# yahoo/bftkv

Measured on AMD Instinct MI355X. Metric: pgp_rsa2048_signature_verifies_per_sec, higher is better.
Workload: dtype u32; 1 GPU; 64-replica quorum, 10000 RSA-2048 signed writes per GPU (cfg2 of BASELINE.json), 534164 signature packets per GPU, 1.0% corrupt / 0.5% unknown issuer / 0.5% duplicate / 1.0% one-short; parallelism=shard-by-write x1, RCCL all-gather of verdict bitmaps on the verifier's stream, replicas=64, writes_per_gpu=10000, sigs_per_gpu=534164, batches_in_flight=3

## Files before the change

### bftkv_amd/csrc/kernels.hip

```cpp
#include <hip/hip_runtime.h>
#include <stdint.h>

#include "device_types.h"
#include "mont28.h"
#include "u256.h"
#include "hashes.h"

namespace bftkv {

struct ParsedPacket {
  uint64_t next;
  bool event;
  SigRec rec;
};

__host__ __device__ __forceinline__ bool known_tag(uint32_t tag) {
  return tag < 32 && ((0x00066BFEu >> tag) & 1u);
}

struct SubpacketState {
  bool have_ctime = false, have_issuer = false, have_embedded = false;
  bool too_deep = false;
  uint64_t issuer = 0;
};
// ... 829 lines not shown
    if (which == 0) sha224_init(s); else if (which == 1) sha1_init(s); else if (which == 4) md5_init(s); else ripemd160_init(s);
    for (uint64_t blk = 0; blk < (len >> 6); ++blk) {
      uint32_t w[16];
      if (which >= 4) { load_block_le(p + blk * 64, w); if (which == 4) md5_compress(s, w); else ripemd160_compress(s, w); }
      else { load_block_be(p + blk * 64, w); if (which == 0) sha256_compress(s, w); else sha1_compress(s, w); }
    }
    const uint32_t slot32 = which < 2 ? which + 1 : which - 1;
    uint32_t* o = mid32 + ((uint64_t)slot32 * n_items + item) * 8;
#pragma unroll
    for (int i = 0; i < 8; ++i) o[i] = s[i];
  } else {
    uint64_t s[8];
    if (which == 2) sha512_init(s); else sha384_init(s);
    for (uint64_t blk = 0; blk < (len >> 7); ++blk) {
      uint32_t lo[16], hi[16];
      load_block_be(p + blk * 128, lo);
      load_block_be(p + blk * 128 + 64, hi);
      uint64_t w[16];
#pragma unroll
      for (int i = 0; i < 8; ++i) { w[i] = ((uint64_t)lo[2 * i] << 32) | lo[2 * i + 1]; w[8 + i] = ((uint64_t)hi[2 * i] << 32) | hi[2 * i + 1]; }
      sha512_compress(s, w);
    }
    uint64_t* o = mid64 + ((uint64_t)(which - 2) * n_items + item) * 8;
#pragma unroll
    for (int i = 0; i < 8; ++i) o[i] = s[i];
  }
}

__global__ void __launch_bounds__(64) k_hash_mid_text(const uint8_t* __restrict__ tbs_blob, const uint64_t* __restrict__ tbs_off,
                                                      uint32_t n_items, const uint32_t* __restrict__ item_hash_mask, TextDev txt) {
  const uint32_t item = blockIdx.x * blockDim.x + threadIdx.x;
  const uint32_t which = blockIdx.y;
  if (item >= n_items) return;
  if (!((item_hash_mask[item] >> (ITEM_TEXT_SHIFT + which)) & 1u)) return;
  const uint8_t* p = tbs_blob + tbs_off[item];
  const uint64_t len = tbs_off[item + 1] - tbs_off[item];
  const bool wide = which == 3 || which == 4;
  const uint32_t B = wide ? 128u : 64u;
  uint32_t s32[8];
  uint64_t s64[8];
  if (which == 0) sha256_init(s32); else if (which == 1) sha224_init(s32); else if (which == 2) sha1_init(s32);
  else if (which == 3) sha512_init(s64); else if (which == 4) sha384_init(s64); else if (which == 5) md5_init(s32); else ripemd160_init(s32);
  uint8_t buf[128];
  uint32_t fill = 0;
  uint64_t total = 0;
  auto put = [&](uint8_t c) {
    buf[fill++] = c;
    ++total;
    if (fill == B) {
      if (which >= 5) {
        uint32_t w[16];
#pragma unroll
        for (int i = 0; i < 16; ++i) w[i] = (uint32_t)buf[4 * i] | ((uint32_t)buf[4 * i + 1] << 8) | ((uint32_t)buf[4 * i + 2] << 16) | ((uint32_t)buf[4 * i + 3] << 24);
        if (which == 5) md5_compress(s32, w); else ripemd160_compress(s32, w);
      } else if (!wide) {
        uint32_t w[16];
#pragma unroll
        for (int i = 0; i < 16; ++i) w[i] = ((uint32_t)buf[4 * i] << 24) | ((uint32_t)buf[4 * i + 1] << 16) | ((uint32_t)buf[4 * i + 2] << 8) | buf[4 * i + 3];
        if (which == 2) sha1_compress(s32, w); else sha256_compress(s32, w);
      } else {
        uint64_t w[16];
#pragma unroll
        for (int i = 0; i < 16; ++i) {
          uint64_t v = 0;
#pragma unroll
          for (int t = 0; t < 8; ++t) v = (v << 8) | buf[8 * i + t];
          w[i] = v;
        }
        sha512_compress(s64, w);
      }
      fill = 0;
    }
  };
  int st = 0;
  for (uint64_t i = 0; i < len; ++i) {
    const uint8_t c = p[i];
    if (st == 0) {
      if (c == 0x0D) { st = 1; put(c); }
      else if (c == 0x0A) { put(0x0D); put(0x0A); }
      else put(c);
    } else { st = 0; put(c); }
  }
  const uint64_t slot = (uint64_t)which * n_items + item;
  if (!wide) {
    const uint32_t slot32 = which < 3 ? which : which - 2;
    for (int i = 0; i < 8; ++i) txt.mid32[((uint64_t)slot32 * n_items + item) * 8 + i] = s32[i];
  } else { for (int i = 0; i < 8; ++i) txt.mid64[((uint64_t)(which - 3) * n_items + item) * 8 + i] = s64[i]; }
  for (uint32_t i = 0; i < fill; ++i) txt.tail[slot * 128 + i] = buf[i];
  txt.len[slot] = total;
}

struct TailSrc {
  const uint8_t* tail; uint32_t tail_len;
  const uint8_t* body; uint32_t pre_len;
  uint32_t tr_len;
  uint32_t rep;
};
__device__ __forceinline__ uint32_t tail_byte(const TailSrc& t, uint32_t j) {
  if (j < t.tail_len) return t.tail[j];
  j -= t.tail_len;
  const uint32_t unit = t.pre_len + t.tr_len;
  if (j >= unit * t.rep) return (j == unit * t.rep) ? 0x80 : 0;
  if (t.rep > 1) j %= unit;
  if (j < t.pre_len) return t.body[j];
  j -= t.pre_len;
  if (j == 0) return 0x04;
  if (j == 1) return 0xFF;
  return (t.pre_len >> (8 * (5 - j))) & 0xFF;
}

template <typename F>
__device__ __forceinline__ uint32_t limb28(F byte_from_lsb, int j) {
  uint32_t bit = 28u * (uint32_t)j;
  uint32_t b0 = bit >> 3, sh = bit & 7;
  uint64_t v = 0;
#pragma unroll
  for (int t = 0; t < 5; ++t) v |= (uint64_t)byte_from_lsb(b0 + t) << (8 * t);
  return (uint32_t)(v >> sh) & MONT_MASK;
}

template <bool OTHERS>
__device__ __forceinline__ void digest_body(const uint8_t* __restrict__ tbs_blob, const uint64_t* __restrict__ tbs_off,
                                            const uint8_t* __restrict__ sig_blob, const uint32_t* __restrict__ mid32,
                                            const uint64_t* __restrict__ mid64, uint32_t n_items,
                                            SigRec* __restrict__ recs, uint32_t n_recs, uint32_t* __restrict__ digests ,
                                            uint32_t ri_in, const uint64_t* __restrict__ tbs_prefix = nullptr, uint32_t rep = 1,
                                            uint32_t* __restrict__ tag_only = nullptr, TextDev txt = TextDev{nullptr, nullptr, nullptr, nullptr}) {
  const uint32_t ri = ri_in;
  if (ri >= n_recs) return;
  const SigRec rec = recs[ri];
  if (!tag_only && rec.status != ST_PENDING_HASH) return;
  const bool text = OTHERS && (rec.flags & SIGF_TEXT) != 0;
  if (!tag_only && ((rec.hash_id != HASH_SHA256) || (rec.flags & SIGF_TEXT) != 0) != OTHERS) return;
  if (OTHERS && text && !txt.len) return;
  const HashInfo hi = OTHERS ? hash_info(rec.hash_id) : HashInfo{32, 0, 32, 19};
  const uint64_t seg = tbs_off[rec.item + 1] - tbs_off[rec.item];
  const uint32_t bmask = (OTHERS && hi.family == 64) ? 127u : 63u;
  const uint64_t tslot = (uint64_t)hi.idx * n_items + rec.item;
  const uint64_t tlen = text ? txt.len[tslot] : (tbs_prefix ? tbs_prefix[rec.item] + seg : seg);
  TailSrc ts;
  ts.tail_len = text ? (uint32_t)(tlen & bmask) : (tbs_prefix ? (uint32_t)seg : (uint32_t)(tlen & bmask));
  ts.tail = text ? txt.tail + tslot * 128 : tbs_blob + tbs_off[rec.item] + (seg - ts.tail_len);
  const bool v3 = (rec.flags & SIGF_V3) != 0;
  ts.body = sig_blob + rec.body_off + (v3 ? 2 : 0);
  ts.pre_len = v3 ? 5u : 6u + rec.hashed_len;
  ts.tr_len = v3 ? 0u : 6u;
  ts.rep = rep;
  const uint32_t rem = ts.tail_len + (ts.pre_len + ts.tr_len) * rep;
  const uint64_t bits = (tlen + (uint64_t)(ts.pre_len + ts.tr_len) * rep) * 8;
  uint32_t dg_dummy[16];
  uint32_t* dg = tag_only ? dg_dummy : digests + (uint64_t)ri * 16;
  uint32_t tag_hi;
  if (!OTHERS || hi.family == 32) {
    const uint32_t nblk = (rem + 9 + 63) >> 6;
    uint32_t s[8];
    const uint32_t* m = (text ? txt.mid32 : mid32) + ((uint64_t)hi.slot * n_items + rec.item) * 8;
#pragma unroll
    for (int i = 0; i < 8; ++i) s[i] = m[i];
    const bool le = OTHERS && hi.le;
    for (uint32_t blk = 0; blk < nblk; ++blk) {
      uint32_t w[16];
#pragma unroll
      for (int i = 0; i < 16; ++i) {
        uint32_t j = blk * 64 + i * 4;
        const uint32_t be = (tail_byte(ts, j) << 24) | (tail_byte(ts, j + 1) << 16) | (tail_byte(ts, j + 2) << 8) | tail_byte(ts, j + 3);
        w[i] = le ? __builtin_bswap32(be) : be;
      }
      if (blk == nblk - 1) { w[14] = le ? (uint32_t)bits : (uint32_t)(bits >> 32); w[15] = le ? (uint32_t)(bits >> 32) : (uint32_t)bits; }
      if (OTHERS && hi.slot == 2) sha1_compress(s, w);
      else if (OTHERS && hi.slot == 3) md5_compress(s, w);
      else if (OTHERS && hi.slot == 4) ripemd160_compress(s, w);
      else sha256_compress(s, w);
    }
#pragma unroll
    for (int i = 0; i < 8; ++i) dg[i] = le ? s[i] : __builtin_bswap32(s[i]);
    tag_hi = le ? __builtin_bswap32(s[0]) : s[0];
  } else if (OTHERS) {
    const uint32_t nblk = (rem + 17 + 127) >> 7;
    uint64_t s[8];
    const uint64_t* m = (text ? txt.mid64 : mid64) + ((uint64_t)hi.slot * n_items + rec.item) * 8;
#pragma unroll
    for (int i = 0; i < 8; ++i) s[i] = m[i];
    for (uint32_t blk = 0; blk < nblk; ++blk) {
      uint64_t w[16];
#pragma unroll
      for (int i = 0; i < 16; ++i) {
        uint32_t j = blk * 128 + i * 8;
        uint64_t v = 0;
#pragma unroll
        for (int t = 0; t < 8; ++t) v = (v << 8) | tail_byte(ts, j + t);
        w[i] = v;
      }
      if (blk == nblk - 1) { w[14] = 0; w[15] = bits; }
      sha512_compress(s, w);
    }
#pragma unroll
    for (int i = 0; i < 8; ++i) { dg[2 * i] = __builtin_bswap32((uint32_t)(s[i] >> 32)); dg[2 * i + 1] = __builtin_bswap32((uint32_t)s[i]); }
    tag_hi = (uint32_t)(s[0] >> 32);
  } else {
    tag_hi = 0;
  }
  if (tag_only) { *tag_only = tag_hi >> 16; return; }
  uint8_t st;
  if ((uint8_t)(tag_hi >> 24) != rec.hash_tag[0] || (uint8_t)(tag_hi >> 16) != rec.hash_tag[1]) st = ST_HASH_TAG;
  else st = (rec.after_tag == AFTER_TAG_PUBKEY) ? (uint8_t)ST_PENDING_RSA : rec.after_tag;
  recs[ri].status = st;
}

__global__ void __launch_bounds__(256) k_digest_sha256(const uint8_t* __restrict__ tbs_blob, const uint64_t* __restrict__ tbs_off,
                                                       const uint8_t* __restrict__ sig_blob, const uint32_t* __restrict__ mid32,
                                                       const uint64_t* __restrict__ mid64, uint32_t n_items, SigRec* __restrict__ recs,
                                                       uint32_t n_recs, uint32_t* __restrict__ digests,
                                                       const uint64_t* __restrict__ tbs_prefix, const uint32_t* __restrict__ n_recs_dev) {
  digest_body<false>(tbs_blob, tbs_off, sig_blob, mid32, mid64, n_items, recs, n_recs_dev ? *n_recs_dev : n_recs, digests,
                     blockIdx.x * blockDim.x + threadIdx.x, tbs_prefix);
}
__global__ void __launch_bounds__(256) k_digest_other(const uint8_t* __restrict__ tbs_blob, const uint64_t* __restrict__ tbs_off,
                                                         const uint8_t* __restrict__ sig_blob, const uint32_t* __restrict__ mid32,
                                                         const uint64_t* __restrict__ mid64, uint32_t n_items, SigRec* __restrict__ recs,
                                                         uint32_t n_recs, uint32_t* __restrict__ digests,
                                                         const uint32_t* __restrict__ any_other , TextDev txt,
                                                         const uint32_t* __restrict__ n_recs_dev ) {
  if (*any_other == 0) return;
  if (n_recs_dev) n_recs = *n_recs_dev;
  for (uint64_t ri = (uint64_t)blockIdx.x * blockDim.x + threadIdx.x; ri < n_recs; ri += (uint64_t)gridDim.x * blockDim.x)
    digest_body<true>(tbs_blob, tbs_off, sig_blob, mid32, mid64, n_items, recs, n_recs, digests, (uint32_t)ri, nullptr, 1, nullptr, txt);
}

__global__ void __launch_bounds__(64) k_candidates(const uint8_t* __restrict__ tbs_blob, const uint64_t* __restrict__ tbs_off,
                                                   const uint8_t* __restrict__ sig_blob, const uint32_t* __restrict__ mid32,
                                                   const uint64_t* __restrict__ mid64, uint32_t n_items, SigRec* __restrict__ recs,
                                                   uint32_t n_recs, const uint32_t* __restrict__ n_recs_dev, const uint64_t* __restrict__ tbs_prefix,
                                                   KeyTableDev kt, const uint32_t* __restrict__ cert_ent, const uint8_t* __restrict__ sig_class,
                                                   TextDev txt, uint32_t* __restrict__ item_hash_mask) {
  const uint32_t ri = blockIdx.x * blockDim.x + threadIdx.x;
  const uint32_t nr = n_recs_dev ? *n_recs_dev : n_recs;
  if (ri >= nr) return;
  const SigRec rec = recs[ri];
  if (!(rec.flags & SIGF_MORE_CANDIDATES)) return;
  uint8_t st = rec.status;
  if (!(st == ST_KEY_CANNOT_SIGN || st == ST_HASH_TAG || st == ST_ALGO_MISMATCH || st == ST_BAD_SIG)) return;
  if (tbs_prefix && (rec.hash_id != HASH_SHA256 || (rec.flags & SIGF_TEXT))) return;
  const uint32_t slot = (uint32_t)rec.key_slot;
  const uint64_t issuer = kt.key_id[slot];
  const uint32_t only_ent = cert_ent ? cert_ent[rec.item] : 0xFFFFFFFFu;
  const uint32_t cls = sig_class ? sig_class[rec.item] : 0;
  uint32_t lo_i = 0, hi_i = kt.n_keys;
  while (lo_i < hi_i) {
    const uint32_t mid = (lo_i + hi_i) >> 1;
    if (kt.sorted_id[mid] < issuer) lo_i = mid + 1; else hi_i = mid;
  }
  bool behind = false;
  uint32_t writes = (kt.flags[slot] & KEYF_CAN_SIGN) ? 1u : 0u;
  for (uint32_t i = lo_i; i < kt.n_keys && kt.sorted_id[i] == issuer; ++i) {
    const uint32_t k = kt.sorted_slot[i];
    if (!key_is_candidate(kt, k, only_ent, cls)) continue;
    if (k == slot) { behind = true; continue; }
    if (!behind) continue;
    if (!(kt.flags[k] & KEYF_CAN_SIGN)) { st = ST_KEY_CANNOT_SIGN; continue; }
    ++writes;
    uint32_t tag = 0;
    if (rec.hash_id == HASH_SHA256 && !(rec.flags & SIGF_TEXT))
      digest_body<false>(tbs_blob, tbs_off, sig_blob, mid32, mid64, n_items, recs, nr, nullptr, ri, tbs_prefix, writes, &tag);
    else digest_body<true>(tbs_blob, tbs_off, sig_blob, mid32, mid64, n_items, recs, nr, nullptr, ri, tbs_prefix, writes, &tag, txt);
    if ((uint8_t)(tag >> 8) != rec.hash_tag[0] || (uint8_t)tag != rec.hash_tag[1]) st = ST_HASH_TAG;
    else if (kt.pk_algo[k] != rec.pk_algo) st = ST_ALGO_MISMATCH;
    else {
      st = ST_BAD_SIG;
      atomicOr(&item_hash_mask[rec.item], ITEM_FENCED);
    }
  }
  recs[ri].status = st;
}

constexpr int RSA_BLOCK = 256;
constexpr int QUADS_PER_BLOCK = RSA_BLOCK / MONT_TPI;
#ifndef BFTKV_MODEXP_BLOCK
#define BFTKV_MODEXP_BLOCK 256
#endif
constexpr int MODEXP_BLOCK = BFTKV_MODEXP_BLOCK;

enum : int { OP_TO_MONT = 0, OP_SQR = 1, OP_MULX = 2, OP_MULP = 3, OP_MUL1 = 4 };

constexpr int EM_LOW_BYTES = 84;
constexpr int EM_LOW_LIMBS = EM_LOW_BYTES * 8 / MONT_W;
static_assert(EM_LOW_LIMBS * MONT_W == EM_LOW_BYTES * 8, "the EM split must fall on a limb boundary");
constexpr uint32_t EM_HEAD_BAD = 0xFFFFFFFFu;

__device__ __forceinline__ uint32_t em_head_limb(uint32_t gi, uint32_t kbytes) {
  const int32_t top = 8 * ((int32_t)kbytes - 2), lo = (int32_t)gi * MONT_W;
  if (top < lo) return 0u;
  if (top >= lo + MONT_W - 1) return MONT_MASK;
  return (1u << (top - lo + 1)) - 1u;
}

template <int L, int TPI>
__global__ void __launch_bounds__(MODEXP_BLOCK, 3) k_rsa_modexp(const uint8_t* __restrict__ sig_blob, const SigRec* __restrict__ recs,
                                                          const uint32_t* __restrict__ pk_list, const uint32_t* __restrict__ pk_count_ptr,
                                                          const uint32_t* __restrict__ pk_start_ptr,
                                                          KeyTableDev kt, uint32_t* __restrict__ r_low,
                                                          uint32_t* __restrict__ xr_scratch, uint64_t* __restrict__ clk) {
  constexpr int NL = TPI * L;
  constexpr int GROUPS = MODEXP_BLOCK / TPI;
  const bool stamp = clk && blockIdx.x == 0 && threadIdx.x == 0;
  uint64_t t0 = 0, r0 = 0;
  if (stamp) { t0 = __builtin_readcyclecounter(); r0 = __builtin_amdgcn_s_memrealtime(); }
  __shared__ uint32_t a_sh[GROUPS * NL];
  __shared__ uint32_t x_sh[GROUPS * NL];
  const uint32_t count = *pk_count_ptr, start = *pk_start_ptr;
  if (start + blockIdx.x * GROUPS >= count) return;
  const uint32_t quad = threadIdx.x / TPI;
  const int qlane = threadIdx.x % TPI;
  const uint32_t gq = start + blockIdx.x * GROUPS + quad;
  const bool active = gq < count;
  const uint32_t pi = active ? gq : (count - 1);
  const uint32_t ri = pk_list[pi];
  const SigRec rec = recs[ri];
  const uint32_t key = (uint32_t)rec.key_slot;
  uint32_t* a_lds = a_sh + quad * NL + qlane * L;
  const uint32_t* a_rd = a_sh + quad * NL;
  uint32_t* x_lds = x_sh + quad * NL + qlane * L;

  uint32_t n[L], b[L], y[L];
  const uint32_t* np = kt.n_limbs + (uint64_t)key * MONT_NMAX + qlane * L;
  const uint32_t* rp = (L == 10 && TPI == 8) ? kt.r2_limbs80 + (uint64_t)key * 80 + qlane * L
                                              : kt.r2_limbs + (uint64_t)key * MONT_NMAX + qlane * L;
  uint32_t* xrp = xr_scratch + (uint64_t)pi * NL + qlane * L;
#pragma unroll
  for (int k = 0; k < L; ++k) n[k] = np[k];
  {
    const uint32_t nb = (rec.mpi_bits[0] + 7u) >> 3;
    const uint8_t* mp = sig_blob + rec.body_off + rec.mpi_off[0];
    auto sig_b = [&](uint32_t i) -> uint32_t { return i < nb ? mp[nb - 1 - i] : 0u; };
#pragma unroll
    for (int k = 0; k < L; ++k) x_lds[k] = limb28(sig_b, qlane * L + k);
  }
  const uint32_t n0inv = kt.n0inv[key];
  const uint32_t e = kt.rsa_e[key];
  const uint32_t kbytes = (kt.mod_bits[key] + 7) >> 3;
  const uint32_t cls = (e << 1) | (((e & 1u) && e > 1u && !(rec.flags & 1u)) ? 1u : 0u);

  uint64_t todo = __builtin_amdgcn_ballot_w64(true);
  while (todo) {
    const int lead = __builtin_ctzll(todo);
    const uint32_t cls_u = (uint32_t)__builtin_amdgcn_readlane((int)cls, lead);
    const bool live = (cls == cls_u);
    const uint32_t e_u = cls_u >> 1;
    const bool sc_u = cls_u & 1u;
    const int top = 31 - __builtin_clz(e_u | 1u);
    int kind = OP_TO_MONT, bitpos = top;
    while (true) {
      if (kind == OP_TO_MONT) {
#pragma unroll
        for (int k = 0; k < L; ++k) { b[k] = rp[k]; a_lds[k] = x_lds[k]; }
      } else {
#pragma unroll
        for (int k = 0; k < L; ++k) b[k] = y[k];
        if (kind == OP_SQR) {
#pragma unroll
          for (int k = 0; k < L; ++k) a_lds[k] = y[k];
        } else if (kind == OP_MULX) {
#pragma unroll
          for (int k = 0; k < L; ++k) a_lds[k] = xrp[k];
        } else if (kind == OP_MULP) {
#pragma unroll
          for (int k = 0; k < L; ++k) a_lds[k] = x_lds[k];
        } else {
#pragma unroll
          for (int k = 0; k < L; ++k) a_lds[k] = (qlane == 0 && k == 0) ? 1u : 0u;
        }
      }
      __builtin_amdgcn_fence(__ATOMIC_ACQ_REL, "wavefront");
      if (kind == OP_SQR) mont_mul<L, TPI, true>(y, a_rd, b, n, n0inv, qlane);
      else mont_mul<L, TPI, false>(y, a_rd, b, n, n0inv, qlane);
      __builtin_amdgcn_fence(__ATOMIC_ACQ_REL, "wavefront");
      if (kind == OP_TO_MONT && (e_u & (e_u - 1u)) != 0 && !(sc_u && __builtin_popcount(e_u) == 2)) {
#pragma unroll
        for (int k = 0; k < L; ++k) xrp[k] = y[k];
      }
      if (kind == OP_MULP || kind == OP_MUL1) break;
      if (kind == OP_SQR && ((e_u >> bitpos) & 1u)) { kind = (bitpos == 0 && sc_u) ? OP_MULP : OP_MULX; continue; }
      --bitpos;
      kind = (bitpos >= 0) ? OP_SQR : OP_MUL1;
    }
    canonicalize<L, TPI>(y, qlane);
    if (e_u == 0) {
#pragma unroll
      for (int k = 0; k < L; ++k) y[k] = (qlane == 0 && k == 0) ? 1u : 0u;
    }
    uint32_t head = 0;
#pragma unroll
    for (int k = 0; k < L; ++k) {
      const uint32_t gi = (uint32_t)qlane * L + k;
      if (gi >= (uint32_t)EM_LOW_LIMBS) head |= y[k] ^ em_head_limb(gi, kbytes);
    }
    head = grp_or<TPI>(head);
    if (head != 0 && qlane == 0) y[0] = EM_HEAD_BAD;
#pragma unroll
    for (int k = 0; k < L; ++k) a_lds[k] = y[k];
    __builtin_amdgcn_fence(__ATOMIC_ACQ_REL, "wavefront");
    if (live && active && qlane < 4) {
      uint32_t* out = r_low + (uint64_t)pi * EM_LOW_LIMBS + qlane * (EM_LOW_LIMBS / 4);
      const uint32_t* src = a_rd + qlane * (EM_LOW_LIMBS / 4);
#pragma unroll
      for (int k = 0; k < EM_LOW_LIMBS / 4; ++k) out[k] = src[k];
    }
    __builtin_amdgcn_fence(__ATOMIC_ACQ_REL, "wavefront");
    todo &= ~__builtin_amdgcn_ballot_w64(live);
  }
  if (stamp && *pk_start_ptr == 0) { clk[0] = __builtin_readcyclecounter() - t0; clk[1] = __builtin_amdgcn_s_memrealtime() - r0; }
}

constexpr int CMP_LANES = 4;
constexpr int CMP_L = EM_LOW_LIMBS / CMP_LANES;
static_assert(CMP_L * CMP_LANES == EM_LOW_LIMBS, "the low limbs divide over the quad");
__global__ void __launch_bounds__(256) k_rsa_compare(SigRec* __restrict__ recs, const uint32_t* __restrict__ pk_list,
                                                     const uint32_t* __restrict__ pk_count_ptr, const uint32_t* __restrict__ pk_start_ptr,
                                                     KeyTableDev kt,
                                                     const uint32_t* __restrict__ r_low, const uint32_t* __restrict__ digests) {
  constexpr int GROUPS = 256 / CMP_LANES;
  const uint32_t count = *pk_count_ptr, start = *pk_start_ptr;
  const uint32_t q0 = start + blockIdx.x * GROUPS;
  if (q0 >= count) return;
  const uint32_t gq = q0 + threadIdx.x / CMP_LANES;
  const int qlane = threadIdx.x % CMP_LANES;
  const bool active = gq < count;
  const uint32_t pi = active ? gq : (count - 1);
  const uint32_t ri = pk_list[pi];
  const SigRec rec = recs[ri];
  const bool pending = rec.status == ST_PENDING_RSA;
  const uint32_t key = (uint32_t)rec.key_slot;
  const uint32_t kbytes = (kt.mod_bits[key] + 7) >> 3;
  const HashInfo hi = hash_info(rec.hash_id);
  const uint32_t hlen = hi.dlen, plen = hi.plen, tl = hlen + plen;
  constexpr int EM_TAIL_W = 24;
  __shared__ uint32_t tail_sh[GROUPS * EM_TAIL_W];
  uint32_t* tail = tail_sh + (threadIdx.x / CMP_LANES) * EM_TAIL_W;
  const uint32_t* dgw = digests + (uint64_t)ri * 16;
  const uint32_t hw = hlen >> 2;
#pragma unroll
  for (int t = 0; t < EM_TAIL_W / CMP_LANES; ++t) {
    const uint32_t w = (uint32_t)qlane * (EM_TAIL_W / CMP_LANES) + t;
    uint32_t v = 0;
    if (w < hw) v = __builtin_bswap32(dgw[hw - 1 - w]);
    else {
#pragma unroll
      for (uint32_t bq = 0; bq < 4; ++bq) {
        const uint32_t i = 4 * w + bq;
        if (i >= hlen && i < tl) v |= digestinfo_byte(rec.hash_id, plen - 1 - (i - hlen)) << (8 * bq);
      }
    }
    tail[w] = v;
  }
  __builtin_amdgcn_fence(__ATOMIC_ACQ_REL, "wavefront");
  auto em_word = [&](uint32_t w) -> uint32_t {
    if (4 * w + 3 <= tl) return tail[w];
    if (4 * w > tl && 4 * w + 3 + 2 < kbytes) return 0xFFFFFFFFu;
    uint32_t v = 0;
#pragma unroll
    for (uint32_t bq = 0; bq < 4; ++bq) {
      const uint32_t i = 4 * w + bq;
      uint32_t byte;
      if (i <= tl) byte = (tail[i >> 2] >> (8 * (i & 3))) & 0xFFu;
      else if (i + 2 < kbytes) byte = 0xFF;
      else byte = (i + 2 == kbytes) ? 1u : 0u;
      v |= byte << (8 * bq);
    }
    return v;
  };
  constexpr int NW = (CMP_L * MONT_W + 31) / 32 + 1;
  const uint32_t bit0 = (uint32_t)qlane * CMP_L * MONT_W, w0 = bit0 >> 5, s0 = bit0 & 31u;
  uint32_t Wd[NW + 1], Wn[NW];
#pragma unroll
  for (int i = 0; i <= NW; ++i) Wd[i] = em_word(w0 + i);
#pragma unroll
  for (int i = 0; i < NW; ++i) Wn[i] = __builtin_amdgcn_alignbit(Wd[i + 1], Wd[i], s0);
  __shared__ uint32_t r_sh[GROUPS * EM_LOW_LIMBS];
  {
    const uint32_t n_valid = min((uint32_t)GROUPS, count - q0) * EM_LOW_LIMBS;
    const uint32_t* src = r_low + (uint64_t)q0 * EM_LOW_LIMBS;
    for (uint32_t t = threadIdx.x; t < GROUPS * EM_LOW_LIMBS; t += 256) r_sh[t] = t < n_valid ? src[t] : 0u;
    __syncthreads();
  }
  const uint32_t* rp = r_sh + (threadIdx.x / CMP_LANES) * EM_LOW_LIMBS + qlane * CMP_L;
  uint32_t diff = 0;
#pragma unroll
  for (int k = 0; k < CMP_L; ++k) {
    const int bit = MONT_W * k, wi = bit >> 5, sh = bit & 31;
    const uint32_t em = (sh == 0 ? Wn[wi] : __builtin_amdgcn_alignbit(Wn[wi + 1], Wn[wi], sh)) & MONT_MASK;
    diff |= em ^ rp[k];
  }
  diff = quad_or(diff);
  if (active && pending && qlane == 0) recs[ri].status = (diff == 0) ? ST_OK : ST_BAD_SIG;
}

constexpr int DSA_U_WORDS = 24;
__device__ __forceinline__ const uint32_t* dsa_slot_base(const KeyTableDev& kt, uint32_t key) {
  return kt.dsa_comb + (uint64_t)kt.dsa_slot[key] * dsa_slot_stride(kt.dsa_wbits, kt.dsa_entry_limbs);
}
__device__ __forceinline__ const uint32_t* dsa_qconst(const KeyTableDev& kt, uint32_t key) {
  return dsa_slot_base(kt, key) + dsa_comb_limbs_per_key(kt.dsa_wbits, kt.dsa_entry_limbs) + dsa_qpow_words(kt.dsa_entry_limbs);
}
__global__ void __launch_bounds__(64) k_dsa_inv(const uint8_t* __restrict__ sig_blob, const SigRec* __restrict__ recs,
                                                const uint32_t* __restrict__ dsa_list, const uint32_t* __restrict__ pk_count,
                                                const uint32_t* __restrict__ pk_start,
                                                KeyTableDev kt, uint32_t* __restrict__ dsa_u , uint32_t batch_min) {
  if (pk_count[1] - pk_start[1] >= batch_min) return;
  const uint32_t di = pk_start[1] + blockIdx.x * blockDim.x + threadIdx.x;
  if (di >= pk_count[1]) return;
  const uint32_t ri = dsa_list[di];
  const uint32_t key = (uint32_t)recs[ri].key_slot;
  const uint64_t body_off = recs[ri].body_off;
  const uint32_t off0 = recs[ri].mpi_off[0], off1 = recs[ri].mpi_off[1], bits0 = recs[ri].mpi_bits[0], bits1 = recs[ri].mpi_bits[1];
  U256 q, r, s_, w;
  for (int i = 0; i < 8; ++i) q.w[i] = kt.q_words[(uint64_t)key * 8 + i];
  const uint32_t qbits = kt.q_bits[key];
  const uint8_t* body = sig_blob + body_off;
  bool ok = u256_from_be(body + off0, (bits0 + 7u) >> 3, r);
  ok = u256_from_be(body + off1, (bits1 + 7u) >> 3, s_) && ok;
  ok = ok && !u256_is_zero(r) && u256_cmp(r, q) < 0 && !u256_is_zero(s_) && u256_cmp(s_, q) < 0;
  ok = ok && (qbits & 7u) == 0;
  ok = ok && u256_modinv_odd(s_, q, w);
  U256 u2 = u256_zero();
  if (ok) {
    const uint32_t* qc = dsa_qconst(kt, key);
    U256 r2;
    for (int i = 0; i < 8; ++i) r2.w[i] = qc[i];
    u2 = u256_mulmod_mont(w, r, q, qc[8], r2);
  } else w = u256_zero();
  uint32_t* o = dsa_u + (uint64_t)di * DSA_U_WORDS;
  for (int i = 0; i < 8; ++i) { o[i] = w.w[i]; o[8 + i] = u2.w[i]; o[16 + i] = r.w[i]; }
}

constexpr int INV_BLOCK = 256, INV_PER_THREAD = 16, INV_TILE = INV_BLOCK * INV_PER_THREAD, INV_MAX_SLOTS = 4096;
__global__ void __launch_bounds__(INV_BLOCK) k_dsa_inv_batched(const uint8_t* __restrict__ sig_blob, const SigRec* __restrict__ recs,
                                                               const uint32_t* __restrict__ dsa_list, const uint32_t* __restrict__ pk_count,
                                                               const uint32_t* __restrict__ pk_start,
                                                               KeyTableDev kt, uint32_t* __restrict__ dsa_u , uint32_t batch_min) {
  if (pk_count[1] - pk_start[1] < batch_min) return;
  __shared__ uint32_t bins[INV_MAX_SLOTS];
  __shared__ uint32_t tsum[INV_BLOCK];
  __shared__ uint16_t order[INV_TILE], slot_of[INV_TILE];
  const uint32_t count = pk_count[1], start = pk_start[1];
  const uint32_t tile0 = start + blockIdx.x * INV_TILE;
  if (tile0 >= count) return;
  const uint32_t n = min((uint32_t)INV_TILE, count - tile0);
  const uint32_t t = threadIdx.x;
#pragma unroll
  for (int j = 0; j < INV_MAX_SLOTS / INV_BLOCK; ++j) bins[t + INV_BLOCK * j] = 0;
  __syncthreads();
  for (int j = 0; j < INV_PER_THREAD; ++j) {
    const uint32_t e = t + INV_BLOCK * j;
    if (e < n) {
      const uint32_t sl = kt.dsa_slot[(uint32_t)recs[dsa_list[tile0 + e]].key_slot] & (INV_MAX_SLOTS - 1);
      slot_of[e] = (uint16_t)sl;
      atomicAdd(&bins[sl], 1u);
    }
  }
  __syncthreads();
  constexpr int BPT = INV_MAX_SLOTS / INV_BLOCK;
  uint32_t loc[BPT], sum = 0;
#pragma unroll
  for (int j = 0; j < BPT; ++j) { loc[j] = sum; sum += bins[BPT * t + j]; }
  tsum[t] = sum;
  __syncthreads();
  for (uint32_t off = 1; off < INV_BLOCK; off <<= 1) {
    const uint32_t v = t >= off ? tsum[t - off] : 0u;
    __syncthreads();
    tsum[t] += v;
    __syncthreads();
  }
  const uint32_t base = tsum[t] - sum;
#pragma unroll
  for (int j = 0; j < BPT; ++j) bins[BPT * t + j] = base + loc[j];
  __syncthreads();
  for (int j = 0; j < INV_PER_THREAD; ++j) {
    const uint32_t e = t + INV_BLOCK * j;
    if (e < n) order[atomicAdd(&bins[slot_of[e]], 1u)] = (uint16_t)e;
  }
  __syncthreads();
  uint32_t pos = INV_PER_THREAD * t;
  const uint32_t end = min(pos + INV_PER_THREAD, n);
  U256 one = u256_zero();
  one.w[0] = 1;
  while (pos < end) {
    const uint32_t sl = slot_of[order[pos]];
    uint32_t re = pos + 1;
    while (re < end && slot_of[order[re]] == sl) ++re;
    const uint32_t key = (uint32_t)recs[dsa_list[tile0 + order[pos]]].key_slot;
    U256 q, r2;
#pragma unroll
    for (int i = 0; i < 8; ++i) q.w[i] = kt.q_words[(uint64_t)key * 8 + i];
    const uint32_t* qc = dsa_qconst(kt, key);
#pragma unroll
    for (int i = 0; i < 8; ++i) r2.w[i] = qc[i];
    const uint32_t q0inv = qc[8];
    const bool q_ok = (kt.q_bits[key] & 7u) == 0;
    uint32_t valid = 0;
    U256 P = one;
    for (uint32_t i = pos; i < re; ++i) {
      const uint32_t di = tile0 + order[i], ri = dsa_list[di];
      const uint8_t* body = sig_blob + recs[ri].body_off;
      U256 r, s_;
      bool ok = u256_from_be(body + recs[ri].mpi_off[0], (recs[ri].mpi_bits[0] + 7u) >> 3, r);
      ok = u256_from_be(body + recs[ri].mpi_off[1], (recs[ri].mpi_bits[1] + 7u) >> 3, s_) && ok;
      ok = ok && q_ok && !u256_is_zero(r) && u256_cmp(r, q) < 0 && !u256_is_zero(s_) && u256_cmp(s_, q) < 0;
      uint32_t* o = dsa_u + (uint64_t)di * DSA_U_WORDS;
      U256 st = u256_zero(), pw = u256_zero();
      if (ok) {
        st = u256_montmul(s_, r2, q, q0inv);
        P = valid ? u256_montmul(P, st, q, q0inv) : st;
        pw = P;
        valid |= 1u << (i - pos);
      }
#pragma unroll
      for (int k = 0; k < 8; ++k) { o[k] = pw.w[k]; o[8 + k] = st.w[k]; o[16 + k] = r.w[k]; }
    }
    if (valid) {
      U256 inv;
      const bool inv_ok = u256_modinv_odd(u256_montmul(P, one, q, q0inv), q, inv);
      U256 I = u256_montmul(inv, r2, q, q0inv);
      for (uint32_t i = re; i-- > pos;) {
        if (!((valid >> (i - pos)) & 1u)) continue;
        uint32_t* o = dsa_u + (uint64_t)(tile0 + order[i]) * DSA_U_WORDS;
        U256 st, r, w, u2;
#pragma unroll
        for (int k = 0; k < 8; ++k) { st.w[k] = o[8 + k]; r.w[k] = o[16 + k]; }
        if (inv_ok) {
          const uint32_t below = valid & ((1u << (i - pos)) - 1u);
          U256 wt = I;
          if (below) {
            const uint32_t pv = pos + (31u - (uint32_t)__builtin_clz(below));
            const uint32_t* op = dsa_u + (uint64_t)(tile0 + order[pv]) * DSA_U_WORDS;
            U256 Pp;
#pragma unroll
            for (int k = 0; k < 8; ++k) Pp.w[k] = op[k];
            wt = u256_montmul(I, Pp, q, q0inv);
          }
          I = u256_montmul(I, st, q, q0inv);
          w = u256_montmul(wt, one, q, q0inv);
          u2 = u256_montmul(wt, r, q, q0inv);
        } else {
          const bool ok1 = u256_modinv_odd(u256_montmul(st, one, q, q0inv), q, w);
          if (ok1) u2 = u256_mulmod_mont(w, r, q, q0inv, r2);
          else { w = u256_zero(); u2 = u256_zero(); }
        }
#pragma unroll
        for (int k = 0; k < 8; ++k) { o[k] = w.w[k]; o[8 + k] = u2.w[k]; }
      }
    }
    pos = re;
  }
}

__global__ void __launch_bounds__(64) k_dsa_mul(SigRec* __restrict__ recs, const uint32_t* __restrict__ dsa_list,
                                                const uint32_t* __restrict__ pk_count, const uint32_t* __restrict__ pk_start, KeyTableDev kt,
                                                const uint32_t* __restrict__ digests, uint32_t* __restrict__ dsa_u) {
  const uint32_t di = pk_start[1] + blockIdx.x * blockDim.x + threadIdx.x;
  if (di >= pk_count[1]) return;
  const uint32_t ri = dsa_list[di];
  const SigRec rec = recs[ri];
  if (rec.status != ST_PENDING_RSA) return;
  uint32_t* o = dsa_u + (uint64_t)di * DSA_U_WORDS;
  U256 q, w;
  for (int i = 0; i < 8; ++i) { q.w[i] = kt.q_words[(uint64_t)rec.key_slot * 8 + i]; w.w[i] = o[i]; }
  if (u256_is_zero(w)) { recs[ri].status = ST_BAD_SIG; return; }
  const HashInfo hi = hash_info(rec.hash_id);
  const uint32_t zlen = min(hi.dlen, kt.q_bits[rec.key_slot] >> 3);
  U256 z;
  u256_from_be((const uint8_t*)(digests + (uint64_t)ri * 16), zlen, z);
  while (u256_cmp(z, q) >= 0) u256_sub(z, q);
  const uint32_t* qc = dsa_qconst(kt, (uint32_t)rec.key_slot);
  U256 r2;
  for (int i = 0; i < 8; ++i) r2.w[i] = qc[i];
  const U256 u1 = u256_mulmod_mont(w, z, q, qc[8], r2);
  for (int i = 0; i < 8; ++i) o[i] = u1.w[i];
}

template <int L, int TPI>
__global__ void __launch_bounds__(RSA_BLOCK) k_dsa_build_comb(uint32_t n_new, const uint32_t* __restrict__ new_slots ,
                                                              const uint32_t* __restrict__ slot_key ,
                                                              KeyTableDev kt, uint32_t* __restrict__ comb, uint32_t parts) {
  constexpr int NL = L * TPI, GROUPS = RSA_BLOCK / TPI;
  __shared__ uint32_t a_sh[GROUPS * NL];
  const uint32_t E = kt.dsa_entry_limbs;
  const uint32_t wbits = kt.dsa_wbits, nwin = dsa_nwin(wbits), nent = (1u << wbits) - 1u;
  const uint32_t n_quads = n_new * 2u * nwin * parts;
  const uint32_t quad = threadIdx.x / TPI;
  const int qlane = threadIdx.x % TPI;
  const uint32_t gq0 = blockIdx.x * GROUPS + quad;
  const bool active = gq0 < n_quads;
  const uint32_t gq = active ? gq0 : (n_quads - 1);
  const uint32_t part = gq % parts, gw = gq / parts;
  const uint32_t which = gw / (2u * nwin), base = (gw / nwin) & 1u, w = gw % nwin;
  const uint32_t key = slot_key[which];
  uint32_t* a_lds = a_sh + quad * NL + qlane * L;
  const uint32_t* a_rd = a_sh + quad * NL;
  uint32_t n[L], b[L], y[L], t[L], one[L];
  const uint32_t* np = kt.n_limbs + (uint64_t)key * MONT_NMAX + qlane * L;
  const uint32_t* sp = kt.dsa_tab + ((uint64_t)key * 2 + base) * DSA_N_BIG + qlane * L;
  const uint32_t* rp = kt.r2_limbs + (uint64_t)key * MONT_NMAX + qlane * L;
#pragma unroll
  for (int k = 0; k < L; ++k) { n[k] = np[k]; y[k] = sp[k]; }
  const uint32_t n0inv = kt.n0inv[key];
  const uint32_t nsq = wbits * w;
  for (uint32_t i = 0; i < wbits * (nwin - 1); ++i) {
// ... 543 lines not shown
```

### bftkv_amd/csrc/mont28.h

```cpp
#pragma once
#include <hip/hip_runtime.h>
#include <stdint.h>

namespace bftkv {

constexpr int MONT_W = 28;
constexpr uint32_t MONT_MASK = (1u << MONT_W) - 1;
constexpr int MONT_TPI = 4;
constexpr int MONT_L = 19;
constexpr int MONT_N = MONT_TPI * MONT_L;
constexpr int MONT_TPI_BIG = 8;
constexpr int MONT_L3072 = 14, MONT_L4096 = 19;
constexpr int MONT_NMAX = MONT_TPI_BIG * MONT_L4096;

constexpr int DPP_QUAD_BCAST0 = 0x00;
constexpr int DPP_QUAD_SHR1 = 0x90;
constexpr int DPP_QUAD_SWAP1 = 0xB1;
constexpr int DPP_QUAD_SWAP2 = 0x4E;
constexpr int DPP_ROW_SHL1 = 0x101;

__device__ __forceinline__ uint32_t dpp_quad_bcast0(uint32_t v) {
  return (uint32_t)__builtin_amdgcn_update_dpp(0, (int)v, DPP_QUAD_BCAST0, 0xF, 0xF, true);
}
__device__ __forceinline__ uint32_t dpp_quad_shr1(uint32_t v) {
  return (uint32_t)__builtin_amdgcn_update_dpp(0, (int)v, DPP_QUAD_SHR1, 0xF, 0xF, false);
}
__device__ __forceinline__ uint32_t dpp_row_shl1(uint32_t v) {
  return (uint32_t)__builtin_amdgcn_update_dpp(0, (int)v, DPP_ROW_SHL1, 0xF, 0xF, true);
}
constexpr int DPP_ROW_SHR1 = 0x111;
constexpr int DPP_ROW_SHR4 = 0x114;
__device__ __forceinline__ uint32_t dpp_row_shr1(uint32_t v) {
  return (uint32_t)__builtin_amdgcn_update_dpp(0, (int)v, DPP_ROW_SHR1, 0xF, 0xF, true);
}
__device__ __forceinline__ uint32_t dpp_row_shr4(uint32_t v) {
  return (uint32_t)__builtin_amdgcn_update_dpp(0, (int)v, DPP_ROW_SHR4, 0xF, 0xF, true);
}
__device__ __forceinline__ uint32_t quad_or(uint32_t v) {
  v |= (uint32_t)__builtin_amdgcn_update_dpp(0, (int)v, DPP_QUAD_SWAP1, 0xF, 0xF, false);
  v |= (uint32_t)__builtin_amdgcn_update_dpp(0, (int)v, DPP_QUAD_SWAP2, 0xF, 0xF, false);
  return v;
}

template <int TPI>
__device__ __forceinline__ uint32_t grp_bcast0(uint32_t v, int glane) {
  const uint32_t q = dpp_quad_bcast0(v);
  if constexpr (TPI == 4) return q;
  else { const uint32_t u = dpp_row_shr4(q); return (glane & 4) ? u : q; }
}
template <int TPI>
__device__ __forceinline__ uint32_t grp_shr1(uint32_t v) {
  if constexpr (TPI == 4) return dpp_quad_shr1(v);
  else return dpp_row_shr1(v);
}
template <int TPI>
__device__ __forceinline__ uint32_t grp_or(uint32_t v) {
  v = quad_or(v);
  if constexpr (TPI == 8) v |= (uint32_t)__shfl_xor((int)v, 4);
  return v;
}

__device__ __forceinline__ uint64_t mad64(uint32_t a, uint32_t b, uint64_t c) {
  return (uint64_t)a * (uint64_t)b + c;
}

template <int L, int TPI, bool SQR, int O>
__device__ __forceinline__ void mont_block_ring(uint64_t (&Q)[2 * L], const uint32_t* ap, const uint32_t (&b)[L],
                                                const uint32_t (&n)[L], uint32_t n0inv, int qlane, uint32_t mask_v) {
  constexpr int M = 2 * L;
#pragma unroll
  for (int r = 0; r < L; ++r) {
    const uint32_t ai = ap[r];
    const uint32_t ai2 = ai << 1;
    uint64_t in = 0;
    if (r > 0) in = dpp_row_shl1((uint32_t)Q[(O + r - 1) % M]) & mask_v;
#pragma unroll
    for (int k = SQR ? r : 0; k < L; ++k) {
      const uint32_t av = (SQR && k > r) ? ai2 : ai;
      if (k == L - 1 && r > 0) Q[(O + r + k) % M] = mad64(av, b[k], in);
      else Q[(O + r + k) % M] = mad64(av, b[k], Q[(O + r + k) % M]);
    }
    const uint32_t m = grp_bcast0<TPI>((uint32_t)Q[(O + r) % M] * n0inv, qlane) & mask_v;
#pragma unroll
    for (int k = 0; k < L; ++k) Q[(O + r + k) % M] = mad64(m, n[k], Q[(O + r + k) % M]);
    Q[(O + r + 1) % M] += Q[(O + r) % M] >> MONT_W;
  }
  Q[(O + M - 1) % M] = dpp_row_shl1((uint32_t)Q[(O + L - 1) % M]) & mask_v;
}

template <int L, int TPI = MONT_TPI, bool SQR = false>
__device__ __forceinline__ void mont_mul(uint32_t (&out)[L], const uint32_t* a_lds,
                                         const uint32_t (&b)[L], const uint32_t (&n)[L],
                                         uint32_t n0inv, int qlane) {
  constexpr bool NORM = 2 * TPI * L > 255;
  static_assert(TPI % 2 == 0, "the ring window runs two blocks per loop iteration");
  uint32_t mask_v;
  asm("v_mov_b32 %0, 0xfffffff" : "=v"(mask_v));
  uint64_t Q[NORM ? 2 * L - 1 : 2 * L];
#pragma unroll
  for (int k = 0; k < L + (NORM ? 1 : 0); ++k) Q[k] = 0;

  if constexpr (!NORM) {
#pragma unroll 1
    for (int blk = 0; blk < TPI; blk += 2) {
      mont_block_ring<L, TPI, SQR, 0>(Q, a_lds + blk * L, b, n, n0inv, qlane, mask_v);
      mont_block_ring<L, TPI, SQR, L>(Q, a_lds + (blk + 1) * L, b, n, n0inv, qlane, mask_v);
    }
  } else {
#pragma unroll 1
    for (int blk = 0; blk < TPI; ++blk) {
      const uint32_t* ap = a_lds + blk * L;
#pragma unroll
      for (int r = 0; r < L; ++r) {
        const uint32_t ai = ap[r];
        const uint32_t ai2 = ai << 1;
#pragma unroll
        for (int k = SQR ? r : 0; k < L; ++k) {
          const uint32_t av = (SQR && k > r) ? ai2 : ai;
          if (k == L - 1 && r > 0) Q[r + k] = mad64(av, b[k], (r == 1) ? Q[r + k] : 0);
          else Q[r + k] = mad64(av, b[k], Q[r + k]);
        }
        const uint32_t m = grp_bcast0<TPI>((uint32_t)Q[r] * n0inv, qlane) & mask_v;
#pragma unroll
        for (int k = 0; k < L; ++k) Q[r + k] = mad64(m, n[k], Q[r + k]);
        Q[r + 1] += Q[r] >> MONT_W;
      }
#pragma unroll
      for (int k = 0; k < L; ++k) {
        const uint64_t nx = dpp_row_shl1((uint32_t)Q[k]) & mask_v;
        Q[k] = (k < L - 1) ? Q[L + k] + nx : nx;
      }
#pragma unroll
      for (int k = 0; k < L; ++k) {
        const uint64_t c = Q[k] >> MONT_W;
        Q[k] &= MONT_MASK;
        if (k < L - 1) Q[k + 1] += c; else Q[L] = c;
      }
    }
  }

  uint64_t c = 0;
#pragma unroll
  for (int k = 0; k < L; ++k) {
    uint64_t v = Q[k] + c;
    out[k] = (uint32_t)v & MONT_MASK;
    c = v >> MONT_W;
  }
  if (NORM) c += Q[L];
  uint32_t clo = grp_shr1<TPI>((uint32_t)c), chi = grp_shr1<TPI>((uint32_t)(c >> 32));
  uint64_t cin = (qlane == 0) ? 0 : (((uint64_t)chi << 32) | clo);
  uint64_t v0 = (uint64_t)out[0] + cin;
  out[0] = (uint32_t)v0 & MONT_MASK;
  uint32_t v1 = out[1] + (uint32_t)(v0 >> MONT_W);
  out[1] = v1 & MONT_MASK;
  out[2] += v1 >> MONT_W;
}

template <int L, int TPI = MONT_TPI>
__device__ __forceinline__ void canonicalize(uint32_t (&x)[L], int qlane) {
  uint32_t cout = 0;
#pragma unroll
  for (int step = 0; step < TPI; ++step) {
    uint32_t c = grp_shr1<TPI>(cout);
    if (qlane == 0) c = 0;
#pragma unroll
    for (int k = 0; k < L; ++k) {
      uint32_t v = x[k] + c;
      x[k] = v & MONT_MASK;
      c = v >> MONT_W;
    }
    cout = c;
  }
}

template <int L, int TPI = MONT_TPI>
__device__ __forceinline__ void reduce_once(uint32_t (&y)[L], const uint32_t (&n)[L], int qlane) {
  uint32_t ge = 1;
#pragma unroll
  for (int k = 0; k < L; ++k) ge = (y[k] > n[k]) ? 1u : ((y[k] < n[k]) ? 0u : ge);
  if (!__any(ge != 0 && qlane == TPI - 1)) return;
  uint32_t d[L];
#pragma unroll
  for (int k = 0; k < L; ++k) d[k] = y[k] - n[k];
  int32_t cout = 0, top = 0;
#pragma unroll
  for (int step = 0; step < TPI; ++step) {
    int32_t c = (int32_t)grp_shr1<TPI>((uint32_t)cout);
    if (qlane == 0) c = 0;
#pragma unroll
    for (int k = 0; k < L; ++k) {
      const int32_t v = (int32_t)d[k] + c;
      d[k] = (uint32_t)v & MONT_MASK;
      c = v >> MONT_W;
    }
    cout = c;
    top += c;
  }
  uint32_t keep = (top == 0) ? 1u : 0u;
  if constexpr (TPI == 4) keep = (uint32_t)__builtin_amdgcn_update_dpp(0, (int)keep, 0xFF, 0xF, 0xF, true);
  else keep = (uint32_t)__shfl((int)keep, (int)((threadIdx.x & 63u) | (uint32_t)(TPI - 1)));
  if (keep) {
#pragma unroll
    for (int k = 0; k < L; ++k) y[k] = d[k];
  }
}

}
```

Baseline: 153.0 million verifies/s.

## Cut modexp register pressure and store doubled limbs for squaring

The RSA modexp kernel drops the separate y accumulator and computes Montgomery products in place into b. It also stops keeping the signature limbs in a second LDS array; instead it re-reads them from global memory at the to-Montgomery and final-multiply steps. Empty asm barriers force indices and key-derived values to be recomputed near where they are used rather than held live in registers. Squarings now read an LDS operand stored as (a, 2a) pairs, which removes the per-row shift in the inner loop but doubles that buffer's LDS footprint and adds extra global reads of the signature and record data.

Result: no change. 152.9 million verifies/s, median of 2 (-0.0%).

```diff
diff --git a/bftkv_amd/csrc/kernels.hip b/bftkv_amd/csrc/kernels.hip
--- a/bftkv_amd/csrc/kernels.hip
+++ b/bftkv_amd/csrc/kernels.hip
@@ -1155,11 +1155,11 @@
                                                           uint32_t* __restrict__ xr_scratch, uint64_t* __restrict__ clk) {
   constexpr int NL = TPI * L;
   constexpr int GROUPS = MODEXP_BLOCK / TPI;
-  const bool stamp = clk && blockIdx.x == 0 && threadIdx.x == 0;
+  const bool stamp_blk = clk && blockIdx.x == 0;
+  const bool stamp = stamp_blk && threadIdx.x == 0;
   uint64_t t0 = 0, r0 = 0;
-  if (stamp) { t0 = __builtin_readcyclecounter(); r0 = __builtin_amdgcn_s_memrealtime(); }
-  __shared__ uint32_t a_sh[GROUPS * NL];
-  __shared__ uint32_t x_sh[GROUPS * NL];
+  if (stamp_blk) { t0 = __builtin_readcyclecounter(); r0 = __builtin_amdgcn_s_memrealtime(); }
+  __shared__ uint32_t a_sh[GROUPS * 2 * NL];
   const uint32_t count = *pk_count_ptr, start = *pk_start_ptr;
   if (start + blockIdx.x * GROUPS >= count) return;
   const uint32_t quad = threadIdx.x / TPI;
@@ -1170,27 +1170,19 @@
   const uint32_t ri = pk_list[pi];
   const SigRec rec = recs[ri];
   const uint32_t key = (uint32_t)rec.key_slot;
-  uint32_t* a_lds = a_sh + quad * NL + qlane * L;
-  const uint32_t* a_rd = a_sh + quad * NL;
-  uint32_t* x_lds = x_sh + quad * NL + qlane * L;
-
-  uint32_t n[L], b[L], y[L];
+  uint32_t* a_lds = a_sh + quad * 2 * NL + qlane * L;
+  const uint32_t* a_rd = a_sh + quad * 2 * NL;
+
+  uint32_t n[L], b[L];
   const uint32_t* np = kt.n_limbs + (uint64_t)key * MONT_NMAX + qlane * L;
-  const uint32_t* rp = (L == 10 && TPI == 8) ? kt.r2_limbs80 + (uint64_t)key * 80 + qlane * L
-                                              : kt.r2_limbs + (uint64_t)key * MONT_NMAX + qlane * L;
-  uint32_t* xrp = xr_scratch + (uint64_t)pi * NL + qlane * L;
+  auto r2_of = [&](uint32_t key_, uint32_t qlane_) {
+    return (L == 10 && TPI == 8) ? kt.r2_limbs80 + (uint64_t)key_ * 80 + qlane_ * L : kt.r2_limbs + (uint64_t)key_ * MONT_NMAX + qlane_ * L;
+  };
 #pragma unroll
   for (int k = 0; k < L; ++k) n[k] = np[k];
-  {
-    const uint32_t nb = (rec.mpi_bits[0] + 7u) >> 3;
-    const uint8_t* mp = sig_blob + rec.body_off + rec.mpi_off[0];
-    auto sig_b = [&](uint32_t i) -> uint32_t { return i < nb ? mp[nb - 1 - i] : 0u; };
-#pragma unroll
-    for (int k = 0; k < L; ++k) x_lds[k] = limb28(sig_b, qlane * L + k);
-  }
   const uint32_t n0inv = kt.n0inv[key];
   const uint32_t e = kt.rsa_e[key];
-  const uint32_t kbytes = (kt.mod_bits[key] + 7) >> 3;
+  auto here_only = [](uint32_t v) { asm volatile("" : "+v"(v)); return v; };
   const uint32_t cls = (e << 1) | (((e & 1u) && e > 1u && !(rec.flags & 1u)) ? 1u : 0u);
 
   uint64_t todo = __builtin_amdgcn_ballot_w64(true);
@@ -1203,58 +1195,63 @@
     const int top = 31 - __builtin_clz(e_u | 1u);
     int kind = OP_TO_MONT, bitpos = top;
     while (true) {
-      if (kind == OP_TO_MONT) {
-#pragma unroll
-        for (int k = 0; k < L; ++k) { b[k] = rp[k]; a_lds[k] = x_lds[k]; }
+      const uint32_t pi_s = here_only(pi), qlane_s = here_only((uint32_t)qlane);
+      uint32_t* xrp = xr_scratch + (uint64_t)pi_s * NL + qlane_s * L;
+      if (kind == OP_TO_MONT || kind == OP_MULP) {
+        const SigRec& rec_s = recs[pk_list[pi_s]];
+        if (kind == OP_TO_MONT) {
+          const uint32_t* rp = r2_of((uint32_t)rec_s.key_slot, qlane_s);
+#pragma unroll
+          for (int k = 0; k < L; ++k) b[k] = rp[k];
+        }
+        const uint32_t nb_s = (rec_s.mpi_bits[0] + 7u) >> 3;
+        const uint8_t* mp_s = sig_blob + rec_s.body_off + rec_s.mpi_off[0];
+        auto sig_b = [&](uint32_t i) -> uint32_t { const uint32_t v = *(i < nb_s ? mp_s + (nb_s - 1 - i) : sig_blob); return i < nb_s ? v : 0u; };
+#pragma unroll
+        for (int k = 0; k < L; ++k) a_lds[k] = limb28(sig_b, qlane_s * L + k);
+      } else if (kind == OP_SQR) {
+        mont_store_pairs<L>(a_lds + qlane * L, b);
+      } else if (kind == OP_MULX) {
+#pragma unroll
+        for (int k = 0; k < L; ++k) a_lds[k] = xrp[k];
       } else {
 #pragma unroll
-        for (int k = 0; k < L; ++k) b[k] = y[k];
-        if (kind == OP_SQR) {
-#pragma unroll
-          for (int k = 0; k < L; ++k) a_lds[k] = y[k];
-        } else if (kind == OP_MULX) {
-#pragma unroll
-          for (int k = 0; k < L; ++k) a_lds[k] = xrp[k];
-        } else if (kind == OP_MULP) {
-#pragma unroll
-          for (int k = 0; k < L; ++k) a_lds[k] = x_lds[k];
-        } else {
-#pragma unroll
-          for (int k = 0; k < L; ++k) a_lds[k] = (qlane == 0 && k == 0) ? 1u : 0u;
-        }
+        for (int k = 0; k < L; ++k) a_lds[k] = (qlane == 0 && k == 0) ? 1u : 0u;
       }
       __builtin_amdgcn_fence(__ATOMIC_ACQ_REL, "wavefront");
-      if (kind == OP_SQR) mont_mul<L, TPI, true>(y, a_rd, b, n, n0inv, qlane);
-      else mont_mul<L, TPI, false>(y, a_rd, b, n, n0inv, qlane);
+      if (kind == OP_SQR) mont_sqr_pairs<L, TPI>(b, a_rd, b, n, n0inv, qlane);
+      else mont_mul<L, TPI, false>(b, a_rd, b, n, n0inv, qlane);
       __builtin_amdgcn_fence(__ATOMIC_ACQ_REL, "wavefront");
       if (kind == OP_TO_MONT && (e_u & (e_u - 1u)) != 0 && !(sc_u && __builtin_popcount(e_u) == 2)) {
 #pragma unroll
-        for (int k = 0; k < L; ++k) xrp[k] = y[k];
+        for (int k = 0; k < L; ++k) xrp[k] = b[k];
       }
       if (kind == OP_MULP || kind == OP_MUL1) break;
       if (kind == OP_SQR && ((e_u >> bitpos) & 1u)) { kind = (bitpos == 0 && sc_u) ? OP_MULP : OP_MULX; continue; }
       --bitpos;
       kind = (bitpos >= 0) ? OP_SQR : OP_MUL1;
     }
-    canonicalize<L, TPI>(y, qlane);
+    canonicalize<L, TPI>(b, qlane);
     if (e_u == 0) {
 #pragma unroll
-      for (int k = 0; k < L; ++k) y[k] = (qlane == 0 && k == 0) ? 1u : 0u;
-    }
+      for (int k = 0; k < L; ++k) b[k] = (qlane == 0 && k == 0) ? 1u : 0u;
+    }
+    const uint32_t pi_s = here_only(pi), qlane_s = here_only((uint32_t)qlane);
+    const uint32_t kbytes_s = (kt.mod_bits[(uint32_t)recs[pk_list[pi_s]].key_slot] + 7) >> 3;
     uint32_t head = 0;
 #pragma unroll
     for (int k = 0; k < L; ++k) {
-      const uint32_t gi = (uint32_t)qlane * L + k;
-      if (gi >= (uint32_t)EM_LOW_LIMBS) head |= y[k] ^ em_head_limb(gi, kbytes);
+      const uint32_t gi = qlane_s * L + k;
+      if (gi >= (uint32_t)EM_LOW_LIMBS) head |= b[k] ^ em_head_limb(gi, kbytes_s);
     }
     head = grp_or<TPI>(head);
-    if (head != 0 && qlane == 0) y[0] = EM_HEAD_BAD;
-#pragma unroll
-    for (int k = 0; k < L; ++k) a_lds[k] = y[k];
+    if (head != 0 && qlane == 0) b[0] = EM_HEAD_BAD;
+#pragma unroll
+    for (int k = 0; k < L; ++k) a_lds[k] = b[k];
     __builtin_amdgcn_fence(__ATOMIC_ACQ_REL, "wavefront");
     if (live && active && qlane < 4) {
-      uint32_t* out = r_low + (uint64_t)pi * EM_LOW_LIMBS + qlane * (EM_LOW_LIMBS / 4);
-      const uint32_t* src = a_rd + qlane * (EM_LOW_LIMBS / 4);
+      uint32_t* out = r_low + (uint64_t)pi_s * EM_LOW_LIMBS + qlane_s * (EM_LOW_LIMBS / 4);
+      const uint32_t* src = a_rd + qlane_s * (EM_LOW_LIMBS / 4);
 #pragma unroll
       for (int k = 0; k < EM_LOW_LIMBS / 4; ++k) out[k] = src[k];
     }
diff --git a/bftkv_amd/csrc/mont28.h b/bftkv_amd/csrc/mont28.h
--- a/bftkv_amd/csrc/mont28.h
+++ b/bftkv_amd/csrc/mont28.h
@@ -64,14 +64,14 @@
   return (uint64_t)a * (uint64_t)b + c;
 }
 
-template <int L, int TPI, bool SQR, int O>
+template <int L, int TPI, bool SQR, int O, bool A2 = false>
 __device__ __forceinline__ void mont_block_ring(uint64_t (&Q)[2 * L], const uint32_t* ap, const uint32_t (&b)[L],
                                                 const uint32_t (&n)[L], uint32_t n0inv, int qlane, uint32_t mask_v) {
   constexpr int M = 2 * L;
 #pragma unroll
   for (int r = 0; r < L; ++r) {
-    const uint32_t ai = ap[r];
-    const uint32_t ai2 = ai << 1;
+    const uint32_t ai = A2 ? ap[2 * r] : ap[r];
+    const uint32_t ai2 = A2 ? ap[2 * r + 1] : ai << 1;
     uint64_t in = 0;
     if (r > 0) in = dpp_row_shl1((uint32_t)Q[(O + r - 1) % M]) & mask_v;
 #pragma unroll
@@ -88,10 +88,11 @@
   Q[(O + M - 1) % M] = dpp_row_shl1((uint32_t)Q[(O + L - 1) % M]) & mask_v;
 }
 
-template <int L, int TPI = MONT_TPI, bool SQR = false>
-__device__ __forceinline__ void mont_mul(uint32_t (&out)[L], const uint32_t* a_lds,
-                                         const uint32_t (&b)[L], const uint32_t (&n)[L],
-                                         uint32_t n0inv, int qlane) {
+template <int L, int TPI, bool SQR, bool A2>
+__device__ __forceinline__ void mont_mul_core(uint32_t (&out)[L], const uint32_t* a_lds,
+                                              const uint32_t (&b)[L], const uint32_t (&n)[L],
+                                              uint32_t n0inv, int qlane) {
+  static_assert(SQR || !A2, "only a squaring reads a doubled operand");
   constexpr bool NORM = 2 * TPI * L > 255;
   static_assert(TPI % 2 == 0, "the ring window runs two blocks per loop iteration");
   uint32_t mask_v;
@@ -103,17 +104,17 @@
   if constexpr (!NORM) {
 #pragma unroll 1
     for (int blk = 0; blk < TPI; blk += 2) {
-      mont_block_ring<L, TPI, SQR, 0>(Q, a_lds + blk * L, b, n, n0inv, qlane, mask_v);
-      mont_block_ring<L, TPI, SQR, L>(Q, a_lds + (blk + 1) * L, b, n, n0inv, qlane, mask_v);
+      mont_block_ring<L, TPI, SQR, 0, A2>(Q, a_lds + (A2 ? 2 : 1) * blk * L, b, n, n0inv, qlane, mask_v);
+      mont_block_ring<L, TPI, SQR, L, A2>(Q, a_lds + (A2 ? 2 : 1) * (blk + 1) * L, b, n, n0inv, qlane, mask_v);
     }
   } else {
 #pragma unroll 1
     for (int blk = 0; blk < TPI; ++blk) {
-      const uint32_t* ap = a_lds + blk * L;
+      const uint32_t* ap = a_lds + (A2 ? 2 : 1) * blk * L;
 #pragma unroll
       for (int r = 0; r < L; ++r) {
-        const uint32_t ai = ap[r];
-        const uint32_t ai2 = ai << 1;
+        const uint32_t ai = A2 ? ap[2 * r] : ap[r];
+        const uint32_t ai2 = A2 ? ap[2 * r + 1] : ai << 1;
 #pragma unroll
         for (int k = SQR ? r : 0; k < L; ++k) {
           const uint32_t av = (SQR && k > r) ? ai2 : ai;
@@ -156,6 +157,25 @@
   out[2] += v1 >> MONT_W;
 }
 
+template <int L, int TPI = MONT_TPI, bool SQR = false>
+__device__ __forceinline__ void mont_mul(uint32_t (&out)[L], const uint32_t* a_lds,
+                                         const uint32_t (&b)[L], const uint32_t (&n)[L],
+                                         uint32_t n0inv, int qlane) {
+  mont_mul_core<L, TPI, SQR, false>(out, a_lds, b, n, n0inv, qlane);
+}
+
+template <int L, int TPI = MONT_TPI>
+__device__ __forceinline__ void mont_sqr_pairs(uint32_t (&out)[L], const uint32_t* a2_lds,
+                                               const uint32_t (&b)[L], const uint32_t (&n)[L],
+                                               uint32_t n0inv, int qlane) {
+  mont_mul_core<L, TPI, true, true>(out, a2_lds, b, n, n0inv, qlane);
+}
+template <int L>
+__device__ __forceinline__ void mont_store_pairs(uint32_t* a2_lane, const uint32_t (&b)[L]) {
+#pragma unroll
+  for (int k = 0; k < L; ++k) { a2_lane[2 * k] = b[k]; a2_lane[2 * k + 1] = b[k] << 1; }
+}
+
 template <int L, int TPI = MONT_TPI>
 __device__ __forceinline__ void canonicalize(uint32_t (&x)[L], int qlane) {
   uint32_t cout = 0;
```
